# KC-decoder/Multimodal-Brain-Pattern-Identification_XAI

Hardware: AMD Instinct MI355X
Metric: samples/sec train (multimodal SpectrogramCNN+EEGNet fusion, B=64/GPU, 4x128x256 spectro + 10000x19 EEG) (higher is better)
Workload: dtype bf16

## Files before the change

### multimodal-brain-pattern-identification_xai_amd/csrc/conv3x3_mfma.hip

```cpp
#include <stdlib.h>
#include "bx_common.h"
#include <string.h>

typedef __attribute__((ext_vector_type(8))) short bf16x8;
typedef __attribute__((ext_vector_type(4))) float f32x4;
typedef unsigned int u32x4 __attribute__((ext_vector_type(4)));
typedef unsigned int u32x2 __attribute__((ext_vector_type(2)));

static inline int mfma_ck(int Ci) { return Ci < 64 ? Ci : 64; }
static inline int mfma_ks(int ck) { return (9 * ck + 31) / 32; }

int bx_conv3x3_mfma_supported(int Ci, int Co, int dtype) {
  if (dtype != BX_BF16) return 0;
  if (!(Ci == 8 || Ci == 16 || Ci == 32 || (Ci >= 64 && Ci % 64 == 0))) return 0;
  return (Co >= 16 && Co % 16 == 0) || (Co == 8 && (Ci == 16 || Ci == 32));
}
static inline int mfma_ow(int O_p) { return O_p < 16 ? 16 : O_p; }
extern "C" size_t bx_conv3x3_packed_mfma_bytes(int I_p, int O_p) {
  if (!bx_conv3x3_mfma_supported(I_p, O_p, BX_BF16)) return 0;
  const int ck = mfma_ck(I_p);
  return (size_t)(I_p / ck) * mfma_ks(ck) * mfma_ow(O_p) * 32 * sizeof(bf16_t);
}

__global__ void k_pack_mfma(const float* __restrict__ w, bf16_t* __restrict__ wp, int Cout, int Cin, int I_p, int O_p, int tf,
// ... 128 lines not shown
  BX_REQUIRE((src_nchw || src_slot) && dst_nhwc_bf16, "bx_conv3x3_pack_layout_ex: needs a source (pointer or device slot) and a destination");
  BX_REQUIRE(B > 0 && C > 0 && H > 0 && W > 0 && Cp % 8 == 0 && C <= Cp, "bx_conv3x3_pack_layout_ex: Cp must be a multiple of 8 and >= C");
  const long long HW = (long long)H * W;
  const long long nbx = (HW + 255) / 256;
  BX_REQUIRE(HW < (1ll << 31) && nbx * B + total_blocks < (1ll << 31), "bx_conv3x3_pack_layout_ex: input too large");
  hipLaunchKernelGGL(k_pack_mfma_many, dim3((unsigned)(total_blocks + nbx * B)), dim3(256), 0, (hipStream_t)stream, jobs_device, njobs,
                     total_blocks, src_slot ? (const float*)dst_nhwc_bf16  : src_nchw,
                     (bf16_t*)dst_nhwc_bf16, C, Cp, (int)HW, (int)nbx, (uint64_t*)nullptr, (uint64_t*)nullptr, (uint64_t*)nullptr,
                     (uint64_t*)nullptr, src_slot);
  BX_CHECK_LAUNCH("bx_conv3x3_pack_layout_ex");
  return BX_OK;
}
extern "C" int bx_conv3x3_pack_many_step(const bxPackJob* jobs_device, int njobs, int total_blocks, const float* src_nchw, void* dst_nhwc_bf16,
                                         int B, int C, int H, int W, int Cp, uint64_t* state_a, uint64_t* out_a, uint64_t* state_b,
                                         uint64_t* out_b, bxStream stream) {
  BX_REQUIRE(jobs_device && njobs > 0 && total_blocks > 0, "bx_conv3x3_pack_many_step: bad arguments");
  BX_REQUIRE((src_nchw == nullptr) == (dst_nhwc_bf16 == nullptr), "bx_conv3x3_pack_many_step: src and dst go together");
  BX_REQUIRE(state_a && out_a && state_b && out_b && state_a != state_b, "bx_conv3x3_pack_many_step: four seed pointers, two distinct states");
  long long HW = 0, nbx = 1, extra = 0;
  if (src_nchw) {
    BX_REQUIRE(B > 0 && C > 0 && H > 0 && W > 0 && Cp % 8 == 0 && C <= Cp, "bx_conv3x3_pack_many_step: Cp must be a multiple of 8 and >= C");
    HW = (long long)H * W;
    nbx = (HW + 255) / 256;
    extra = nbx * B;
    BX_REQUIRE(HW < (1ll << 31) && extra + total_blocks < (1ll << 31), "bx_conv3x3_pack_many_step: input too large");
  }
  hipLaunchKernelGGL(k_pack_mfma_many, dim3((unsigned)(total_blocks + extra)), dim3(256), 0, (hipStream_t)stream, jobs_device, njobs,
                     total_blocks, src_nchw, (bf16_t*)dst_nhwc_bf16, C, Cp, (int)HW, (int)nbx, state_a, out_a, state_b, out_b);
  BX_CHECK_LAUNCH("bx_conv3x3_pack_many_step");
  return BX_OK;
}

struct WgradRedJob { const float* partial; float* dw; float* db; int nsplit, Cin, Co, S, MA, NB, ztiles, nfrag4, nblocks; };
__device__ __forceinline__ void wgrad_reduce3_body(const WgradRedJob& jb, int bid, float4* sm);
static WgradRedJob wgrad_job_from(const bxWgradPending* pd, bool chained);
#define BX_WGRAD_RED_MAX 3
struct WgradRedList { WgradRedJob job[BX_WGRAD_RED_MAX]; };
__device__ __forceinline__ void wgrad_reduce_list(const WgradRedList& rl, int bid, float4* sm);

template <int CK>
__device__ __forceinline__ int lds_chunk(int c, int p) {
  if (CK == 32) return c ^ ((p >> 1) & 3);
  if (CK == 64) return c ^ (p & 7);
  return c;
}

__device__ __forceinline__ unsigned char relu_bits(u32x2 v) {
  const uint32_t h[4] = {v.x & 0xffffu, v.x >> 16, v.y & 0xffffu, v.y >> 16};
  unsigned b = 0;
#pragma unroll
  for (int r = 0; r < 4; ++r) b |= (h[r] != 0u && h[r] < 0x8000u) ? (1u << r) : 0u;
  return (unsigned char)b;
}
template <int CTRL> __device__ __forceinline__ float dpp16(float v) {
  return __int_as_float(__builtin_amdgcn_update_dpp(0, __float_as_int(v), CTRL, 0xf, 0xf, false));
}
__device__ __forceinline__ float row16_sum(float v) {
  v += dpp16<0xB1>(v); v += dpp16<0x4E>(v); v += dpp16<0x124>(v); v += dpp16<0x128>(v);
  return v;
}
template <int MP, int NC, int TPR, typename PixFn>
__device__ __forceinline__ void conv_pool_tiles(const f32x4 (&q)[MP][NC], const BxConvPoolEpi& pe, const __amdgpu_buffer_rsrc_t& pres, int Co,
                                                int co_base, PixFn pix, float (&st)[2][NC][4]) {
  const int lane = threadIdx.x & 63, g = lane >> 4, li = lane & 15;
  const __amdgpu_buffer_rsrc_t rres = __builtin_amdgcn_make_buffer_rsrc(pe.route, 0, pe.route ? pe.route_bytes : 0u, 0x00020000);
#pragma unroll
// ... 68 lines not shown
  if (bx_stat_tree_arrive<2>(pe.tree, blockIdx.y, co_base, blockIdx.x, val, tot, lds) && (int)threadIdx.x < CW)
    bx_bn_finalize_channel(co_base + threadIdx.x, tot[0], tot[1], pe.fin);
}
__device__ __forceinline__ void conv_pool_transpose_w1x1(const BxConvPoolEpi& pe, int C) {
  const int nw = pe.Cin1_p * C, nwg = (int)(gridDim.x * gridDim.y), wg = (int)(blockIdx.y * gridDim.x + blockIdx.x);
  const int per = (nw + nwg - 1) / nwg, lo = wg * per, hi = lo + per < nw ? lo + per : nw;
  for (int i = lo + (int)threadIdx.x; i < hi; i += 256) {
    const int ci = i / C, c = i - ci * C;
    pe.wT[i] = ci < pe.Cin1 ? pe.w1x1[(size_t)c * pe.Cin1 + ci] : 0.f;
  }
}

#ifdef BX_CONV_STAMPS
__device__ unsigned long long bx_conv_stamps[64 * 8];
extern "C" int bx_debug_conv_stamps(unsigned long long* host_out) {
  return hipMemcpyFromSymbol(host_out, HIP_SYMBOL(bx_conv_stamps), sizeof(unsigned long long) * 64 * 8) == hipSuccess ? 0 : -1;
}
#define BX_CSTAMP(i) do { if (cstamp_wg >= 0 && threadIdx.x == 0) bx_conv_stamps[cstamp_wg * 8 + (i)] = __builtin_amdgcn_s_memtime(); } while (0)
#else
#define BX_CSTAMP(i) do { } while (0)
#endif
template <int CK, int NC, int TW, int IMGS = 1, bool POOL = false, bool C8 = false, bool W22 = false>
__global__ __launch_bounds__(256) void k_conv_mfma(const bf16_t* __restrict__ x, const bf16_t* __restrict__ wp, const float* __restrict__ bias,
    const bf16_t* __restrict__ mask_src, const bf16_t* __restrict__ addend, bf16_t* __restrict__ y,
    int H, int W, int Ci, int Co, int relu, int tiles_x, int tiles_y, uint32_t x_bytes, BxConvPoolEpi pe, WgradRedList red, int nred) {
  constexpr int TH = 8, HWID = TW + 2, HH = TH + 2, CKB = CK * 2, NCH = CK / 8, KS = (9 * CK + 31) / 32;
  constexpr int MP = (W22 ? 2 : 1) * IMGS * TH * TW / 64;
  constexpr int NCW = W22 ? NC / 2 : NC;
  static_assert(!W22 || (NC % 2 == 0 && !POOL && !C8), "2 x 2 wave grid: even NC, plain epilogue");
  constexpr int TPI = TH * TW / 16;
  constexpr int TPR = TW / 16;
  extern __shared__ __attribute__((aligned(16))) char lds[];
  if ((int)blockIdx.x < nred) {
    if (blockIdx.y == 0) wgrad_reduce_list(red, (int)blockIdx.x, reinterpret_cast<float4*>(lds));
    return;
  }
  const int bid = (int)blockIdx.x - nred;
  const int gx = (int)gridDim.x - nred;
#ifdef BX_CONV_STAMPS
  const int cstamp_lin = (int)(blockIdx.y * gridDim.x + blockIdx.x);
  const int cstamp_wg = (cstamp_lin % 4 == 1 && cstamp_lin / 4 < 64) ? cstamp_lin / 4 : -1;
#endif
  BX_CSTAMP(0);
  const int tx = bid % tiles_x, ty = (bid / tiles_x) % tiles_y, b = (bid / (tiles_x * tiles_y)) * IMGS;
  const int wave = threadIdx.x >> 6, lane = threadIdx.x & 63, g = lane >> 4, li = lane & 15;
  const int wpix = W22 ? wave >> 1 : wave;
  const int y0 = ty * TH, x0 = tx * TW, co_base = blockIdx.y * (NC * 16) + (W22 ? (wave & 1) * NCW * 16 : 0);
  if (POOL) conv_pool_transpose_w1x1(pe, Co);

  f32x4 acc[MP][NCW];
#pragma unroll
  for (int i = 0; i < MP; ++i)
#pragma unroll
    for (int n = 0; n < NCW; ++n) acc[i][n] = (f32x4){0.f, 0.f, 0.f, 0.f};

  const int nchunk = Ci / CK;
  const int Cw = C8 ? 16 : Co;
  constexpr int NU = IMGS * HH * HWID * NCH, NR = (NU + 255) / 256;
  const __amdgpu_buffer_rsrc_t xres = __builtin_amdgcn_make_buffer_rsrc((void*)x, 0, x_bytes, 0x00020000);
  uint32_t hoff[NR];
#pragma unroll
  for (int k = 0; k < NR; ++k) {
    const int u = threadIdx.x + k * 256;
    const int p = u / NCH, c = u % NCH;
    const int img = p / (HH * HWID), pl = p - img * (HH * HWID);
    const int iy = y0 + pl / HWID - 1, ix = x0 + pl % HWID - 1;
    const bool ok = u < NU && (unsigned)iy < (unsigned)H && (unsigned)ix < (unsigned)W;
// ... 333 lines not shown
    for (int n = 0; n < NCW; ++n) {
      float v[4] = {acc[i][n][0] + bz[n].x, acc[i][n][1] + bz[n].y, acc[i][n][2] + bz[n].z, acc[i][n][3] + bz[n].w};
      if (relu) {
#pragma unroll
        for (int r = 0; r < 4; ++r) v[r] = fmaxf(v[r], 0.f);
      }
      if (mask_src) {
        const u32x2 m = mk[i][n];
        const uint32_t mm[4] = {m.x & 0xffffu, m.x >> 16, m.y & 0xffffu, m.y >> 16};
#pragma unroll
        for (int r = 0; r < 4; ++r) v[r] = (mm[r] != 0u && mm[r] < 0x8000u) ? v[r] : 0.f;
      }
      if (addend) {
        const u32x2 a2 = ad[i][n];
        v[0] += __uint_as_float(a2.x << 16); v[1] += __uint_as_float(a2.x & 0xffff0000u);
        v[2] += __uint_as_float(a2.y << 16); v[3] += __uint_as_float(a2.y & 0xffff0000u);
      }
      const u32x2 out = {pack2bf(v[0], v[1]), pack2bf(v[2], v[3])};
      __builtin_amdgcn_raw_buffer_store_b64(out, yres, offs[i] + (uint32_t)(n * 32), 0, 0);
    }
  }
  BX_CSTAMP(6);
}

template <int CK, int NC, int TW, bool POOL = false, bool C8 = false>
__global__ __launch_bounds__(256, (CK == 16 && NC == 1 && TW == 32 && !POOL) ? 4 : 1) void k_conv_mfma_p(const bf16_t* __restrict__ x, const bf16_t* __restrict__ wp, const float* __restrict__ bias,
    const bf16_t* __restrict__ mask_src, const bf16_t* __restrict__ addend, bf16_t* __restrict__ y,
    int H, int W, int Co, int relu, int tiles_x, int tiles_y, int ntiles, uint32_t x_bytes, BxConvPoolEpi pe, WgradRedList red, int nred) {
  constexpr int TH = 8, HWID = TW + 2, HH = TH + 2, CKB = CK * 2, NCH = CK / 8, KS = (9 * CK + 31) / 32;
  constexpr int MP = TH * TW / 64, TPR = TW / 16;
  constexpr int NU = HH * HWID * NCH, NR = (NU + 255) / 256;
  extern __shared__ __attribute__((aligned(16))) char lds[];
  if ((int)blockIdx.x < nred) {
    if (blockIdx.y == 0) wgrad_reduce_list(red, (int)blockIdx.x, reinterpret_cast<float4*>(lds));
    return;
  }
  const int first_tile = (int)blockIdx.x - nred, tile_stride = (int)gridDim.x - nred;
  const int co_base = blockIdx.y * (NC * 16);
  const int wave = threadIdx.x >> 6, lane = threadIdx.x & 63, g = lane >> 4, li = lane & 15;
  uint4 rv[NR];
  const __amdgpu_buffer_rsrc_t xres = __builtin_amdgcn_make_buffer_rsrc((void*)x, 0, x_bytes, 0x00020000);
  int hpy[NR], hpx[NR];
  uint32_t hrel[NR];
#pragma unroll
  for (int k = 0; k < NR; ++k) {
    const int u = threadIdx.x + k * 256;
    const int p = u / NCH, c = u % NCH;
    hpy[k] = u < NU ? p / HWID - 1 : -100000;
    hpx[k] = p % HWID - 1;
    hrel[k] = (uint32_t)(((p / HWID - 1) * W + (p % HWID - 1)) * CK + c * 8) * 2u;
  }
  auto fetch = [&](int tile) {
    const int tx = tile % tiles_x, ty = (tile / tiles_x) % tiles_y, b = tile / (tiles_x * tiles_y);
    const int y0 = ty * TH, x0 = tx * TW;
    const uint32_t tbase = (uint32_t)(((b * H + y0) * W + x0) * CK) * 2u;
#pragma unroll
    for (int k = 0; k < NR; ++k) {
      const bool ok = (unsigned)(y0 + hpy[k]) < (unsigned)H && (unsigned)(x0 + hpx[k]) < (unsigned)W;
      const uint32_t off = ok ? tbase + hrel[k] : 0x80000000u;
      const u32x4 v = __builtin_amdgcn_raw_buffer_load_b128(xres, off, 0, 0);
      rv[k] = make_uint4(v.x, v.y, v.z, v.w);
    }
  };
  const uint32_t y_bytes = (uint32_t)((size_t)(ntiles / (tiles_x * tiles_y)) * H * W * Co * 2);
  const __amdgpu_buffer_rsrc_t yres = __builtin_amdgcn_make_buffer_rsrc((void*)y, 0, y_bytes, 0x00020000);
  const bool mbits = (relu & 2) != 0;
  const __amdgpu_buffer_rsrc_t mres = __builtin_amdgcn_make_buffer_rsrc((void*)(mask_src ? mask_src : y), 0, mbits ? y_bytes / 8 : y_bytes, 0x00020000);
// ... 441 lines not shown
  if (y1)
    hipLaunchKernelGGL((k_conv12_mfma<true>), dim3((unsigned)gx), dim3(256), lds, (hipStream_t)stream, (const bf16_t*)x, (const bf16_t*)packed1_mfma, bias1,
                       (const bf16_t*)packed2_mfma, bias2, (bf16_t*)y1, (bf16_t*)y2, mask1, mask2, H, W, tiles_x, tiles_y, (int)ntiles, xb);
  else
    hipLaunchKernelGGL((k_conv12_mfma<false>), dim3((unsigned)gx), dim3(256), lds, (hipStream_t)stream, (const bf16_t*)x, (const bf16_t*)packed1_mfma, bias1,
                       (const bf16_t*)packed2_mfma, bias2, (bf16_t*)nullptr, (bf16_t*)y2, (unsigned char*)nullptr, (unsigned char*)nullptr, H, W, tiles_x, tiles_y, (int)ntiles, xb);
  BX_CHECK_LAUNCH("bx_conv3x3_pair");
  return BX_OK;
}

template <int NC>
static int pool_tree_shape(BxConvPoolEpi* pe, int grid_x, int ygroups, int Co) {
  pe->tree.nrows = grid_x; pe->tree.Cw = NC * 16; pe->tree.ld = Co;
  bx_stat_tree_shape(grid_x, &pe->tree.G, &pe->tree.ngroups);
  if (!pe->want_stats) return BX_OK;
  if (grid_x > pe->tree_max_rows) pe->tree.cnt = nullptr;
  BX_REQUIRE((size_t)grid_x * 2 * Co <= pe->rows_cap_floats, "bx_conv3x3(pooled): %d partial rows exceed the workspace", grid_x);
  BX_REQUIRE(!pe->tree.cnt || ygroups * (pe->tree.ngroups + 1) <= pe->cnt_cap_words, "bx_conv3x3(pooled): %d x %d reduction groups exceed the sync words",
             ygroups, pe->tree.ngroups);
  return BX_OK;
}
static int wgrad_red_total(const WgradRedList& rl) {
  int n = 0;
  for (int i = 0; i < BX_WGRAD_RED_MAX; ++i) n += rl.job[i].nblocks;
  return n;
}
template <int CK, int NC, int TW>
static int launch_conv(const void* x, const void* wp, const float* bias, const void* mask, const void* addend, void* y,
                       int B, int H, int W, int Ci, int Co, int relu, hipStream_t s, BxConvPoolEpi* pe = nullptr, const WgradRedList* red = nullptr) {
  const int tiles_x = (W + TW - 1) / TW, tiles_y = (H + 7) / 8;
  size_t lds = (size_t)10 * (TW + 2) * CK * 2;
  const BxConvPoolEpi none = {};
  const WgradRedList nored = {};
  const int nred = red && !pe ? wgrad_red_total(*red) : 0;
  const WgradRedList& rj = nred ? *red : nored;
  if (nred && lds < 4096) lds = 4096;
  if (pe) {
    const size_t need = BX_STAT_TREE_LDS(2) + (size_t)4 * 2 * NC * 16 * sizeof(float);
    if (lds < need) lds = need;
  }
  if (Co < 16) {
    if constexpr (NC == 1 && (CK == 16 || CK == 32)) {
      BX_REQUIRE(Co == 8 && Ci == CK && !pe && !bias, "bx_conv3x3(mfma): the 8-channel output form is a plain data gradient (Ci=%d Co=%d)", Ci, Co);
      const int ntiles = tiles_x * tiles_y * B;
      const int gx = ntiles < 2048 ? ntiles : 2048;
      if (ntiles >= 4 * gx && (size_t)B * H * W * CK * 2 < ((size_t)1 << 31)) {
        hipLaunchKernelGGL((k_conv_mfma_p<CK, 1, TW, false, true>), dim3((unsigned)(gx + nred), 1u), dim3(256), lds, s, (const bf16_t*)x,
                           (const bf16_t*)wp, bias, (const bf16_t*)mask, (const bf16_t*)addend, (bf16_t*)y, H, W, Co, relu, tiles_x, tiles_y, ntiles,
                           (uint32_t)((size_t)B * H * W * CK * 2), none, rj, nred);
        BX_CHECK_LAUNCH("bx_conv3x3(mfma persistent, 8 output channels)");
        return BX_OK;
      }
      hipLaunchKernelGGL((k_conv_mfma<CK, 1, TW, 1, false, true>), dim3((unsigned)(ntiles + nred), 1u), dim3(256), lds, s, (const bf16_t*)x,
                         (const bf16_t*)wp, bias, (const bf16_t*)mask, (const bf16_t*)addend, (bf16_t*)y, H, W, Ci, Co, relu, tiles_x, tiles_y,
                         (uint32_t)((size_t)B * H * W * Ci * 2), none, rj, nred);
      BX_CHECK_LAUNCH("bx_conv3x3(mfma, 8 output channels)");
      return BX_OK;
    }
    BX_FAIL(BX_EUNSUPPORTED, "bx_conv3x3(mfma): %d output channels with Ci=%d", Co, Ci);
  }
  if constexpr (CK <= 32) if (Ci == CK) {
    const int ntiles = tiles_x * tiles_y * B, ygroups = Co / (16 * NC);
    constexpr int pgx = 2048, pmin = 4;
    int gx = pgx / ygroups;
    if (gx > ntiles) gx = ntiles;
    if (ntiles >= pmin * gx && (size_t)B * H * W * CK * 2 < ((size_t)1 << 31)) {
      if (pe) {
        if constexpr (CK >= 16) {
          const int rc = pool_tree_shape<NC>(pe, gx, ygroups, Co);
          if (rc != BX_OK) return rc;
          hipLaunchKernelGGL((k_conv_mfma_p<CK, NC, TW, true>), dim3((unsigned)gx, (unsigned)ygroups), dim3(256), lds, s, (const bf16_t*)x,
                             (const bf16_t*)wp, bias, (const bf16_t*)nullptr, (const bf16_t*)nullptr, (bf16_t*)y, H, W, Co, 1, tiles_x, tiles_y, ntiles,
                             (uint32_t)((size_t)B * H * W * CK * 2), *pe, nored, 0);
          BX_CHECK_LAUNCH("bx_conv3x3(mfma persistent, pooled)");
          return BX_OK;
        }
      }
      hipLaunchKernelGGL((k_conv_mfma_p<CK, NC, TW>), dim3((unsigned)(gx + nred), (unsigned)ygroups), dim3(256), lds, s, (const bf16_t*)x,
                         (const bf16_t*)wp, bias, (const bf16_t*)mask, (const bf16_t*)addend, (bf16_t*)y, H, W, Co, relu, tiles_x, tiles_y, ntiles,
                         (uint32_t)((size_t)B * H * W * CK * 2), none, rj, nred);
      BX_CHECK_LAUNCH("bx_conv3x3(mfma persistent)");
      return BX_OK;
    }
  }
  if constexpr (CK == 64) {
    if (tiles_x * tiles_y == 1 && Co >= 256 && B % 2 == 0) {
      const size_t lds2 = lds * 2;
      static bool attr_done = false;
      if (lds2 > 64 * 1024 && !attr_done) {
        if (hipFuncSetAttribute((const void*)k_conv_mfma<CK, NC, TW, 2>, hipFuncAttributeMaxDynamicSharedMemorySize, (int)lds2) != hipSuccess)
          BX_FAIL(BX_EHIP, "bx_conv3x3(mfma): cannot reserve %zu bytes of LDS", lds2);
        attr_done = true;
      }
      dim3 grid2((unsigned)(tiles_x * tiles_y * (B / 2) + nred), (unsigned)(Co / (16 * NC)));
      if (pe) {
        const int rc = pool_tree_shape<NC>(pe, (int)grid2.x, (int)grid2.y, Co);
        if (rc != BX_OK) return rc;
        static bool attr_done_p = false;
        if (lds2 > 64 * 1024 && !attr_done_p) {
          if (hipFuncSetAttribute((const void*)k_conv_mfma<CK, NC, TW, 2, true>, hipFuncAttributeMaxDynamicSharedMemorySize, (int)lds2) != hipSuccess)
            BX_FAIL(BX_EHIP, "bx_conv3x3(mfma): cannot reserve %zu bytes of LDS", lds2);
          attr_done_p = true;
        }
        hipLaunchKernelGGL((k_conv_mfma<CK, NC, TW, 2, true>), grid2, dim3(256), lds2, s, (const bf16_t*)x, (const bf16_t*)wp, bias, (const bf16_t*)nullptr,
                           (const bf16_t*)nullptr, (bf16_t*)y, H, W, Ci, Co, 1, tiles_x, tiles_y, (uint32_t)((size_t)B * H * W * Ci * 2), *pe, nored, 0);
        BX_CHECK_LAUNCH("bx_conv3x3(mfma, two-image tiles, pooled)");
        return BX_OK;
      }
      hipLaunchKernelGGL((k_conv_mfma<CK, NC, TW, 2>), grid2, dim3(256), lds2, s, (const bf16_t*)x, (const bf16_t*)wp, bias, (const bf16_t*)mask,
                         (const bf16_t*)addend, (bf16_t*)y, H, W, Ci, Co, relu, tiles_x, tiles_y, (uint32_t)((size_t)B * H * W * Ci * 2), none, rj, nred);
      BX_CHECK_LAUNCH("bx_conv3x3(mfma, two-image tiles)");
      return BX_OK;
    }
  }
  dim3 grid((unsigned)(tiles_x * tiles_y * B + nred), (unsigned)(Co / (16 * NC)));
  if (pe) {
    if constexpr (CK >= 16) {
      const int rc = pool_tree_shape<NC>(pe, (int)grid.x, (int)grid.y, Co);
      if (rc != BX_OK) return rc;
      hipLaunchKernelGGL((k_conv_mfma<CK, NC, TW, 1, true>), grid, dim3(256), lds, s, (const bf16_t*)x, (const bf16_t*)wp, bias, (const bf16_t*)nullptr,
                         (const bf16_t*)nullptr, (bf16_t*)y, H, W, Ci, Co, 1, tiles_x, tiles_y, (uint32_t)((size_t)B * H * W * Ci * 2), *pe, nored, 0);
      BX_CHECK_LAUNCH("bx_conv3x3(mfma, pooled)");
      return BX_OK;
    }
    BX_FAIL(BX_EUNSUPPORTED, "bx_conv3x3(pooled): needs at least 16 input channels");
  }
  if constexpr (CK == 64 && NC % 2 == 0) {
    hipLaunchKernelGGL((k_conv_mfma<CK, NC, TW, 1, false, false, true>), grid, dim3(256), lds, s, (const bf16_t*)x, (const bf16_t*)wp, bias,
                       (const bf16_t*)mask, (const bf16_t*)addend, (bf16_t*)y, H, W, Ci, Co, relu, tiles_x, tiles_y, (uint32_t)((size_t)B * H * W * Ci * 2), none, rj, nred);
    BX_CHECK_LAUNCH("bx_conv3x3(mfma, 2 x 2 waves)");
  } else {
    hipLaunchKernelGGL((k_conv_mfma<CK, NC, TW>), grid, dim3(256), lds, s, (const bf16_t*)x, (const bf16_t*)wp, bias,
                       (const bf16_t*)mask, (const bf16_t*)addend, (bf16_t*)y, H, W, Ci, Co, relu, tiles_x, tiles_y, (uint32_t)((size_t)B * H * W * Ci * 2), none, rj, nred);
    BX_CHECK_LAUNCH("bx_conv3x3(mfma)");
  }
  return BX_OK;
}
template <int NCW, int TW, int IMGS>
static int launch_conv_c(const void* x, const void* wp, const float* bias, const void* mask, const void* addend, void* y,
                         int B, int H, int W, int Ci, int Co, int relu, hipStream_t s, BxConvPoolEpi* pe) {
  const int tiles_x = (W + TW - 1) / TW, tiles_y = (H + 7) / 8;
  const size_t lds = (size_t)2 * IMGS * 10 * ((TW + 2 + 7) / 8 * 8) * 128;
  dim3 grid((unsigned)(tiles_x * tiles_y * (B / IMGS)), (unsigned)(Co / (64 * NCW)));
  const BxConvPoolEpi none = {};
  auto attr = [&](const void* fn, bool& done) -> int {
    if (lds > 64 * 1024 && !done) {
      if (hipFuncSetAttribute(fn, hipFuncAttributeMaxDynamicSharedMemorySize, (int)lds) != hipSuccess)
// ... 61 lines not shown
  for (int i = 0, k = 0; carry && i < ncarry; ++i)
    if (carry[i].valid) { jobs.job[k++] = wgrad_job_from(&carry[i], true); red = &jobs; }
  BX_REQUIRE((size_t)B * H * W * (Ci > Co ? Ci : Co) * 2 < ((size_t)1 << 31), "bx_conv3x3(mfma): an activation tensor of 2 GiB or more is not supported (B=%d H=%d W=%d)", B, H, W);
  if (!red) {
    const int rc = try_conv_c(x, packed_mfma, bias, relu_mask_src, addend, y, B, H, W, Ci, Co, relu, s, nullptr);
    if (rc >= 0) return rc;
  }
  int rc;
  switch (mfma_ck(Ci)) {
    case 8:  rc = launch_conv_nc<8>(x, packed_mfma, bias, relu_mask_src, addend, y, B, H, W, Ci, Co, relu, s, nullptr, red); break;
    case 16: rc = launch_conv_nc<16>(x, packed_mfma, bias, relu_mask_src, addend, y, B, H, W, Ci, Co, relu, s, nullptr, red); break;
    case 32: rc = launch_conv_nc<32>(x, packed_mfma, bias, relu_mask_src, addend, y, B, H, W, Ci, Co, relu, s, nullptr, red); break;
    default: rc = launch_conv_nc<64>(x, packed_mfma, bias, relu_mask_src, addend, y, B, H, W, Ci, Co, relu, s, nullptr, red); break;
  }
  for (int i = 0; rc == BX_OK && carry && i < ncarry; ++i) carry[i].valid = 0;
  return rc;
}

int bx_conv3x3_mfma_pool_launch(const void* x, const void* packed_mfma, const float* bias, void* y, int B, int H, int W, int Ci, int Co,
                                BxConvPoolEpi* pe, hipStream_t s) {
  BX_REQUIRE((size_t)B * H * W * (Ci > Co ? Ci : Co) * 2 < ((size_t)1 << 31), "bx_conv3x3(pooled): an activation tensor of 2 GiB or more is not supported");
  BX_REQUIRE(Ci >= 16 && pe && pe->pooled, "bx_conv3x3(pooled): needs at least 16 input channels and a pooled output");
  {
    const int rc = try_conv_c(x, packed_mfma, bias, nullptr, nullptr, y, B, H, W, Ci, Co, 1, s, pe);
    if (rc >= 0) return rc;
  }
  switch (mfma_ck(Ci)) {
    case 16: return launch_conv_nc<16>(x, packed_mfma, bias, nullptr, nullptr, y, B, H, W, Ci, Co, 1, s, pe);
    case 32: return launch_conv_nc<32>(x, packed_mfma, bias, nullptr, nullptr, y, B, H, W, Ci, Co, 1, s, pe);
    default: return launch_conv_nc<64>(x, packed_mfma, bias, nullptr, nullptr, y, B, H, W, Ci, Co, 1, s, pe);
  }
}

__device__ __forceinline__ void wgrad_reduce3_body(const WgradRedJob& jb, int bid, float4* sm) {
  const float* __restrict__ partial = jb.partial;
  float* __restrict__ dw = jb.dw;
  float* __restrict__ db = jb.db;
  const int nsplit = jb.nsplit, Cin = jb.Cin, Co = jb.Co, S = jb.S, MA = jb.MA, NB = jb.NB, ztiles = jb.ztiles, nfrag4 = jb.nfrag4;
  const size_t per_split = (size_t)nfrag4 * 4 + Co;
  const int NO = 256 / S;
  const int o = threadIdx.x % NO, part = threadIdx.x / NO;
  const size_t e4 = (size_t)bid * NO + o;
  const bool live = e4 * 4 < per_split;
  float4 s = make_float4(0.f, 0.f, 0.f, 0.f);
  if (live) {
    const float* src = partial + e4 * 4;
    int c = part;
    for (; c + 3 * S < nsplit; c += 4 * S) {
      const float4 v0 = *reinterpret_cast<const float4*>(src + (size_t)c * per_split);
      const float4 v1 = *reinterpret_cast<const float4*>(src + (size_t)(c + S) * per_split);
      const float4 v2 = *reinterpret_cast<const float4*>(src + (size_t)(c + 2 * S) * per_split);
      const float4 v3 = *reinterpret_cast<const float4*>(src + (size_t)(c + 3 * S) * per_split);
      s.x += v0.x; s.y += v0.y; s.z += v0.z; s.w += v0.w;
      s.x += v1.x; s.y += v1.y; s.z += v1.z; s.w += v1.w;
      s.x += v2.x; s.y += v2.y; s.z += v2.z; s.w += v2.w;
      s.x += v3.x; s.y += v3.y; s.z += v3.z; s.w += v3.w;
    }
    for (; c < nsplit; c += S) {
      const float4 v = *reinterpret_cast<const float4*>(src + (size_t)c * per_split);
      s.x += v.x; s.y += v.y; s.z += v.z; s.w += v.w;
    }
  }
  sm[threadIdx.x] = s;
  __syncthreads();
  if (part == 0 && live) {
    float4 r = sm[o];
    for (int k = 1; k < S; ++k) { const float4 v = sm[k * NO + o]; r.x += v.x; r.y += v.y; r.z += v.z; r.w += v.w; }
    const float rr[4] = {r.x, r.y, r.z, r.w};
    if (e4 < (size_t)nfrag4) {
      const int NT = 9 * MA * NB;
      const int lane = (int)(e4 & 63), tl = (int)(e4 >> 6);
      const int i = tl % NT, yz = tl / NT, z = yz % ztiles, y = yz / ztiles;
      const int n = i % NB, m = (i / NB) % MA, t = i / (NB * MA);
      const int cout = (z * NB + n) * 16 + (lane & 15), cin0 = (y * MA + m) * 16 + 4 * (lane >> 4);
#pragma unroll
      for (int j = 0; j < 4; ++j)
        if (cin0 + j < Cin) dw[((size_t)cout * Cin + cin0 + j) * 9 + t] = rr[j];
    } else if (db) {
      const size_t b0 = (e4 - nfrag4) * 4;
#pragma unroll
      for (int j = 0; j < 4; ++j) db[b0 + j] = rr[j];
    }
  }
}
__device__ __forceinline__ void wgrad_reduce_list(const WgradRedList& rl, int bid, float4* sm) {
  if (bid < rl.job[0].nblocks) { wgrad_reduce3_body(rl.job[0], bid, sm); return; }
  bid -= rl.job[0].nblocks;
  if (bid < rl.job[1].nblocks) { wgrad_reduce3_body(rl.job[1], bid, sm); return; }
  bid -= rl.job[1].nblocks;
  if (bid < rl.job[2].nblocks) wgrad_reduce3_body(rl.job[2], bid, sm);
}
__global__ __launch_bounds__(256) void k_wgrad_reduce3(WgradRedJob jb, WgradRedJob jb2) {
  __shared__ float4 sm[256];
  if ((int)blockIdx.x < jb.nblocks) wgrad_reduce3_body(jb, blockIdx.x, sm);
  else wgrad_reduce3_body(jb2, (int)blockIdx.x - jb.nblocks, sm);
}

typedef __attribute__((ext_vector_type(4))) short s16x4;
typedef __attribute__((address_space(3))) s16x4 lds_s16x4;

__device__ __forceinline__ bf16x8 tr_read8(const char* lds, int off0, int off1) {
  const s16x4 lo = __builtin_amdgcn_ds_read_tr16_b64_v4i16((lds_s16x4*)(lds + off0));
  const s16x4 hi = __builtin_amdgcn_ds_read_tr16_b64_v4i16((lds_s16x4*)(lds + off1));
  return (bf16x8){lo[0], lo[1], lo[2], lo[3], hi[0], hi[1], hi[2], hi[3]};
}

template <int MA, int NB, int TW>
__global__ __launch_bounds__(256, 2) void k_wgrad_mfma(const bf16_t* __restrict__ x, const bf16_t* __restrict__ dz, float* __restrict__ partial,
    int H, int W, int Ci_p, int Co, int tiles_x, int tiles_y, int ntiles, int tiles_per_split, WgradRedJob prev, int zextra) {
  constexpr int TH = 8, HWID = TW + 2, HH = TH + 2, CIT = 16 * MA, COT = 16 * NB, XB = CIT * 2, ZB = COT * 2;
  constexpr int KPW = TH * TW / 32 / 4;
  constexpr int XS_BYTES = HH * HWID * XB;
  extern __shared__ __attribute__((aligned(16))) char lds[];
  if ((int)blockIdx.z < zextra) {
    const int rid = ((int)blockIdx.z * (int)gridDim.y + (int)blockIdx.y) * (int)gridDim.x + (int)blockIdx.x;
    if (rid < prev.nblocks) wgrad_reduce3_body(prev, rid, reinterpret_cast<float4*>(lds));
    return;
  }
  const int bz = (int)blockIdx.z - zextra, gz = (int)gridDim.z - zextra;
  char* xs = lds;
  char* zs = lds + XS_BYTES;
  const int wave = threadIdx.x >> 6, lane = threadIdx.x & 63, g = lane >> 4, li = lane & 15;
  const int q = li >> 2, pc = li & 3;
  const int ci0 = blockIdx.y * CIT, co0 = bz * COT;
  const bool want_bias = blockIdx.y == 0;

// ... 348 lines not shown
  wgrad_own_body<TW>(*pj, id - pj->first, lds);
}

struct WgradPlan { int ma, nb, tw, tiles_x, tiles_y, ntiles, ytiles, ztiles, nsplit, tps; size_t lds; };
static WgradPlan wgrad_plan(int B, int H, int W, int Ci_p, int Co) {
  WgradPlan p;
  p.ma = Ci_p >= 32 ? 2 : 1;
  p.nb = Co >= 32 ? 2 : 1;
  p.tw = W <= 16 ? 16 : 32;
  p.tiles_x = (W + p.tw - 1) / p.tw; p.tiles_y = (H + 7) / 8; p.ntiles = p.tiles_x * p.tiles_y * B;
  p.ytiles = (Ci_p + 16 * p.ma - 1) / (16 * p.ma); p.ztiles = Co / (16 * p.nb);
  constexpr int want_wgs = 512;
  int want = want_wgs / (p.ytiles * p.ztiles);
  if (want < 1) want = 1;
  if (want > p.ntiles) want = p.ntiles;
  p.tps = (p.ntiles + want - 1) / want;
  p.nsplit = (p.ntiles + p.tps - 1) / p.tps;
  const size_t stage = (size_t)10 * (p.tw + 2) * 32 * p.ma + (size_t)8 * p.tw * 32 * p.nb;
  const size_t red = (size_t)((9 * p.ma * p.nb + 3) / 4) * 4 * 64 * sizeof(float4);
  p.lds = stage > red ? stage : red;
  return p;
}
int bx_wgrad_mfma_supported(int Ci_p, int Co, int dtype) {
  return dtype == BX_BF16 && Ci_p % 8 == 0 && Co % 16 == 0 && (Co < 32 || Co % 32 == 0) && (Ci_p < 32 || Ci_p % 32 == 0);
}
size_t bx_wgrad_mfma_workspace(int B, int H, int W, int Ci_p, int Co) {
  const WgradPlan p = wgrad_plan(B, H, W, Ci_p, Co);
  return (size_t)p.nsplit * ((size_t)p.ytiles * p.ztiles * 9 * p.ma * p.nb * 256 + Co) * sizeof(float);
}
template <int MA, int NB, int TW>
static void launch_wgrad(const WgradPlan& p, const void* x, const void* dz, float* ws, int H, int W, int Ci_p, int Co, const WgradRedJob& prev,
                         int zextra, hipStream_t s) {
  dim3 grid(p.nsplit, p.ytiles, p.ztiles + zextra);
  hipLaunchKernelGGL((k_wgrad_mfma<MA, NB, TW>), grid, dim3(256), p.lds, s, (const bf16_t*)x, (const bf16_t*)dz, ws, H, W, Ci_p, Co,
                     p.tiles_x, p.tiles_y, p.ntiles, p.tps, prev, zextra);
}
static int wgrad_reduce_slices(size_t per_split, int nsplit, bool chained) {
  if (!chained) return per_split >= 65536 ? 4 : per_split >= 8192 ? 16 : 64;
  int S = 1;
  while (S < 64 && nsplit > 8 * S) S *= 2;
  return S;
}
static WgradRedJob wgrad_job_from(const bxWgradPending* pd, bool chained) {
  WgradRedJob jb;
  jb.partial = (const float*)pd->partial; jb.dw = pd->dw; jb.db = pd->db; jb.nsplit = pd->nsplit; jb.Cin = pd->Cin; jb.Co = pd->Co;
  jb.MA = pd->ma; jb.NB = pd->nb; jb.ztiles = pd->ztiles; jb.nfrag4 = pd->nfrag4;
  const size_t per_split = (size_t)pd->nfrag4 * 4 + pd->Co;
  jb.S = wgrad_reduce_slices(per_split, pd->nsplit, chained);
  const int per_wg = 256 / jb.S;
  jb.nblocks = (int)((per_split / 4 + per_wg - 1) / per_wg);
  return jb;
}
int bx_wgrad_mfma_finish(bxWgradPending* pd, hipStream_t s) {
  if (!pd || !pd->valid) return BX_OK;
  const WgradRedJob jb = wgrad_job_from(pd, false), none = {};
  hipLaunchKernelGGL(k_wgrad_reduce3, dim3(jb.nblocks), dim3(256), 0, s, jb, none);
  pd->valid = 0;
  BX_CHECK_LAUNCH("bx_conv3x3_wgrad(mfma reduce)");
  return BX_OK;
}
int bx_wgrad_mfma_launch(const void* x, const void* dz, float* dw, float* db, int B, int H, int W, int Cin, int Ci_p,
                         int Co, void* ws, size_t ws_bytes, bxWgradPending* pending, hipStream_t s) {
  const WgradPlan p = wgrad_plan(B, H, W, Ci_p, Co);
  (void)ws_bytes;
  BX_REQUIRE((size_t)B * H * W * (Ci_p > Co ? Ci_p : Co) * 2 < ((size_t)1 << 31), "bx_conv3x3_wgrad(mfma): an activation tensor of 2 GiB or more is not supported");
  BX_REQUIRE(!pending || !pending->valid || pending->partial != ws, "bx_conv3x3_wgrad(chained): the pending partials live in this call's workspace");
  float* part = (float*)ws;
  WgradRedJob prev;
  memset(&prev, 0, sizeof(prev));
  int zextra = 0;
  if (pending && pending->valid) {
    prev = wgrad_job_from(pending, true);
    zextra = (prev.nblocks + p.nsplit * p.ytiles - 1) / (p.nsplit * p.ytiles);
  }
  if (p.ma == 2 && p.nb == 2) {
    const int nred = pending && pending->valid ? (prev.nblocks + 7) / 8 * 8 : 0;
    const int ranges8 = (p.nsplit + 7) / 8;
    const int nwg = nred + ranges8 * 8 * p.ytiles * p.ztiles;
    const size_t lds = (size_t)10 * (p.tw + 2) * 64 + (size_t)8 * p.tw * 64 + 256;
    if (p.tw == 16)
      hipLaunchKernelGGL((k_wgrad_own<16, 2>), dim3(nwg), dim3(256), lds, s, (const bf16_t*)x, (const bf16_t*)dz, part, H, W, Ci_p, Co,
                         p.tiles_x, p.tiles_y, p.ntiles, p.tps, p.nsplit, p.ytiles, p.ztiles, prev, nred);
    else
      hipLaunchKernelGGL((k_wgrad_own<32, 2>), dim3(nwg), dim3(256), lds, s, (const bf16_t*)x, (const bf16_t*)dz, part, H, W, Ci_p, Co,
                         p.tiles_x, p.tiles_y, p.ntiles, p.tps, p.nsplit, p.ytiles, p.ztiles, prev, nred);
  } else {
#define BX_WG(MA_, NB_) do { if (p.tw == 16) launch_wgrad<MA_, NB_, 16>(p, x, dz, part, H, W, Ci_p, Co, prev, zextra, s); \
                             else launch_wgrad<MA_, NB_, 32>(p, x, dz, part, H, W, Ci_p, Co, prev, zextra, s); } while (0)
    if (p.ma == 1 && p.nb == 1) BX_WG(1, 1);
    else if (p.ma == 1) BX_WG(1, 2);
    else BX_WG(2, 1);
#undef BX_WG
  }
  BX_CHECK_LAUNCH("bx_conv3x3_wgrad(mfma)");
  bxWgradPending cur;
  cur.partial = part; cur.dw = dw; cur.db = db; cur.nsplit = p.nsplit; cur.Cin = Cin; cur.Co = Co; cur.ma = p.ma; cur.nb = p.nb;
  cur.ztiles = p.ztiles; cur.nfrag4 = p.ytiles * p.ztiles * 9 * p.ma * p.nb * 64; cur.valid = 1;
  if (pending) { *pending = cur; return BX_OK; }
  return bx_wgrad_mfma_finish(&cur, s);
}

static size_t wgrad_group_region(size_t bytes) { return (bytes + 255) / 256 * 256; }
int bx_wgrad_group_supported(int n, const int* Ci_p, const int* Co, int W, int dtype) {
  if (n < 1 || n > BX_WGRAD_GROUP_MAX || !Ci_p || !Co || W <= 0 || dtype != BX_BF16) return 0;
  for (int i = 0; i < n; ++i)
    if (Ci_p[i] < 32 || Co[i] < 32 || !bx_wgrad_mfma_supported(Ci_p[i], Co[i], dtype)) return 0;
  return 1;
}
size_t bx_wgrad_group_workspace(const bxWgradGroupLayer* layers, int n, int B, int H, int W) {
  size_t total = 0;
  for (int i = 0; i < n; ++i) total += wgrad_group_region(bx_wgrad_mfma_workspace(B, H, W, layers[i].Ci_p, layers[i].Co));
  return total;
// ... 246 lines not shown
}

struct FusedBwdPlan { int tiles_x, tiles_y, ntiles, tps, nsplit; };
static FusedBwdPlan fused_bwd_plan(int B, int H, int W) {
  FusedBwdPlan p;
  p.tiles_x = (W + 31) / 32; p.tiles_y = (H + 7) / 8; p.ntiles = p.tiles_x * p.tiles_y * B;
  constexpr int want_wgs = 512;
  const int want = want_wgs < p.ntiles ? want_wgs : p.ntiles;
  p.tps = (p.ntiles + want - 1) / want;
  p.nsplit = (p.ntiles + p.tps - 1) / p.tps;
  return p;
}
extern "C" size_t bx_conv3x3_bwd_fused_workspace(int B, int H, int W, int with_w1) {
  const FusedBwdPlan p = fused_bwd_plan(B, H, W);
  return (size_t)p.nsplit * (9 * 256 + 16) * sizeof(float) * (with_w1 ? 2 : 1);
}
extern "C" int bx_conv3x3_bwd_fused(const void* dz, const void* xl, const void* packed_flip, void* dzo, const void* x0, float* dw, float* db,
                                    float* dw0, float* db0, int B, int H, int W, int Cin0, void* ws, size_t ws_bytes, bxWgradPending* pending,
                                    bxStream stream) {
  hipStream_t s = (hipStream_t)stream;
  const bool w1 = x0 != nullptr;
  BX_REQUIRE(dz && xl && packed_flip && dw && db && ws && B > 0 && H > 0 && W > 0, "bx_conv3x3_bwd_fused: bad arguments");
  BX_REQUIRE(w1 ? (!dzo && dw0 && db0 && Cin0 > 0 && Cin0 <= 8) : (dzo && !dw0 && !db0),
             "bx_conv3x3_bwd_fused: either dzo (data gradient stored) or x0 with dw0 / db0 (conv1's weight gradient, 1..8 input channels)");
  BX_REQUIRE((size_t)B * H * W * 16 * 2 < ((size_t)1 << 31), "bx_conv3x3_bwd_fused: an activation tensor of 2 GiB or more is not supported");
  const FusedBwdPlan p = fused_bwd_plan(B, H, W);
  const size_t need = bx_conv3x3_bwd_fused_workspace(B, H, W, w1);
  BX_REQUIRE(ws_bytes >= need, "bx_conv3x3_bwd_fused: workspace %zu < %zu", ws_bytes, need);
  BX_REQUIRE(!pending || !pending->valid || pending->partial != ws, "bx_conv3x3_bwd_fused: the pending partials live in this call's workspace");
  WgradRedJob prev = {};
  int nred = 0;
  if (pending && pending->valid) { prev = wgrad_job_from(pending, true); nred = prev.nblocks; pending->valid = 0; }
  constexpr int IMG = 10 * 34 * 32;
  const size_t lds = w1 ? (size_t)3 * IMG + 8 * 32 * 32 : (size_t)2 * IMG;
  const uint32_t act_bytes = (uint32_t)((size_t)B * H * W * 16 * 2);
  float* part = (float*)ws;
  if (w1)
    hipLaunchKernelGGL((k_conv_mfma_bwd<true>), dim3((unsigned)(p.nsplit + nred)), dim3(256), lds, s, (const bf16_t*)dz, (const bf16_t*)xl,
                       (const bf16_t*)packed_flip, (const bf16_t*)x0, (bf16_t*)nullptr, part, H, W, p.tiles_x, p.tiles_y, p.ntiles, p.tps, p.nsplit,
                       act_bytes, prev, nred);
  else
    hipLaunchKernelGGL((k_conv_mfma_bwd<false>), dim3((unsigned)(p.nsplit + nred)), dim3(256), lds, s, (const bf16_t*)dz, (const bf16_t*)xl,
                       (const bf16_t*)packed_flip, (const bf16_t*)nullptr, (bf16_t*)dzo, part, H, W, p.tiles_x, p.tiles_y, p.ntiles, p.tps, p.nsplit,
                       act_bytes, prev, nred);
  BX_CHECK_LAUNCH("bx_conv3x3_bwd_fused");
  bxWgradPending cur = {};
  cur.partial = part; cur.dw = dw; cur.db = db; cur.nsplit = p.nsplit; cur.Cin = 16; cur.Co = 16; cur.ma = 1; cur.nb = 1;
  cur.ztiles = 1; cur.nfrag4 = 9 * 64; cur.valid = 1;
  if (!w1) {
    if (pending) { *pending = cur; return BX_OK; }
    return bx_wgrad_mfma_finish(&cur, s);
  }
  bxWgradPending cur0 = cur;
  cur0.partial = part + (size_t)p.nsplit * (9 * 256 + 16); cur0.dw = dw0; cur0.db = db0; cur0.Cin = Cin0;
  const WgradRedJob j1 = wgrad_job_from(&cur, false), j0 = wgrad_job_from(&cur0, false);
  hipLaunchKernelGGL(k_wgrad_reduce3, dim3((unsigned)(j1.nblocks + j0.nblocks)), dim3(256), 0, s, j1, j0);
  BX_CHECK_LAUNCH("bx_conv3x3_bwd_fused(reduce)");
  return BX_OK;
}
```

Before: 48990.

## Reduce wgrad partials per tap triplet and spread reduction blocks across grid y

Adds a new reduction path for small split counts: each thread sums three taps of a fragment position across splits, stages the results in LDS, and then writes dw in the final Co×Ci×3×3 layout with coalesced float4 stores, replacing the old scattered per-element writes. Fused conv launches now spread the chained reduction blocks over every grid-y row instead of only row 0, which shortens the idle x-prefix of the grid. LDS reservations are raised wherever a chained reduction runs. The cost is more LDS per block, which can lower occupancy for small conv kernels, plus extra synchronization inside the reduction.

```diff
diff --git a/multimodal-brain-pattern-identification_xai_amd/csrc/conv3x3_mfma.hip b/multimodal-brain-pattern-identification_xai_amd/csrc/conv3x3_mfma.hip
--- a/multimodal-brain-pattern-identification_xai_amd/csrc/conv3x3_mfma.hip
+++ b/multimodal-brain-pattern-identification_xai_amd/csrc/conv3x3_mfma.hip
@@ -184,6 +184,7 @@
 }
 
 struct WgradRedJob { const float* partial; float* dw; float* db; int nsplit, Cin, Co, S, MA, NB, ztiles, nfrag4, nblocks; };
+#define BX_WGRAD_RED_LDS ((size_t)3 * 256 * sizeof(float4) + (size_t)85 * 36 * sizeof(float))
 __device__ __forceinline__ void wgrad_reduce3_body(const WgradRedJob& jb, int bid, float4* sm);
 static WgradRedJob wgrad_job_from(const bxWgradPending* pd, bool chained);
 #define BX_WGRAD_RED_MAX 3
@@ -318,7 +319,7 @@
   constexpr int TPR = TW / 16;
   extern __shared__ __attribute__((aligned(16))) char lds[];
   if ((int)blockIdx.x < nred) {
-    if (blockIdx.y == 0) wgrad_reduce_list(red, (int)blockIdx.x, reinterpret_cast<float4*>(lds));
+    if constexpr (!POOL) wgrad_reduce_list(red, (int)(blockIdx.y * nred + blockIdx.x), reinterpret_cast<float4*>(lds));
     return;
   }
   const int bid = (int)blockIdx.x - nred;
@@ -718,7 +719,7 @@
   constexpr int NU = HH * HWID * NCH, NR = (NU + 255) / 256;
   extern __shared__ __attribute__((aligned(16))) char lds[];
   if ((int)blockIdx.x < nred) {
-    if (blockIdx.y == 0) wgrad_reduce_list(red, (int)blockIdx.x, reinterpret_cast<float4*>(lds));
+    wgrad_reduce_list(red, (int)(blockIdx.y * nred + blockIdx.x), reinterpret_cast<float4*>(lds));
     return;
   }
   const int first_tile = (int)blockIdx.x - nred, tile_stride = (int)gridDim.x - nred;
@@ -1226,9 +1227,10 @@
   size_t lds = (size_t)10 * (TW + 2) * CK * 2;
   const BxConvPoolEpi none = {};
   const WgradRedList nored = {};
-  const int nred = red && !pe ? wgrad_red_total(*red) : 0;
-  const WgradRedList& rj = nred ? *red : nored;
-  if (nred && lds < 4096) lds = 4096;
+  const int nblk = red && !pe ? wgrad_red_total(*red) : 0;
+  const auto nredx = [nblk](int ny) { return (nblk + ny - 1) / ny; };
+  const WgradRedList& rj = nblk ? *red : nored;
+  if (nblk && lds < BX_WGRAD_RED_LDS) lds = BX_WGRAD_RED_LDS;
   if (pe) {
     const size_t need = BX_STAT_TREE_LDS(2) + (size_t)4 * 2 * NC * 16 * sizeof(float);
     if (lds < need) lds = need;
@@ -1236,7 +1238,7 @@
   if (Co < 16) {
     if constexpr (NC == 1 && (CK == 16 || CK == 32)) {
       BX_REQUIRE(Co == 8 && Ci == CK && !pe && !bias, "bx_conv3x3(mfma): the 8-channel output form is a plain data gradient (Ci=%d Co=%d)", Ci, Co);
-      const int ntiles = tiles_x * tiles_y * B;
+      const int ntiles = tiles_x * tiles_y * B, nred = nredx(1);
       const int gx = ntiles < 2048 ? ntiles : 2048;
       if (ntiles >= 4 * gx && (size_t)B * H * W * CK * 2 < ((size_t)1 << 31)) {
         hipLaunchKernelGGL((k_conv_mfma_p<CK, 1, TW, false, true>), dim3((unsigned)(gx + nred), 1u), dim3(256), lds, s, (const bf16_t*)x,
@@ -1254,7 +1256,7 @@
     BX_FAIL(BX_EUNSUPPORTED, "bx_conv3x3(mfma): %d output channels with Ci=%d", Co, Ci);
   }
   if constexpr (CK <= 32) if (Ci == CK) {
-    const int ntiles = tiles_x * tiles_y * B, ygroups = Co / (16 * NC);
+    const int ntiles = tiles_x * tiles_y * B, ygroups = Co / (16 * NC), nred = nredx(ygroups);
     constexpr int pgx = 2048, pmin = 4;
     int gx = pgx / ygroups;
     if (gx > ntiles) gx = ntiles;
@@ -1286,6 +1288,7 @@
           BX_FAIL(BX_EHIP, "bx_conv3x3(mfma): cannot reserve %zu bytes of LDS", lds2);
         attr_done = true;
       }
+      const int nred = nredx(Co / (16 * NC));
       dim3 grid2((unsigned)(tiles_x * tiles_y * (B / 2) + nred), (unsigned)(Co / (16 * NC)));
       if (pe) {
         const int rc = pool_tree_shape<NC>(pe, (int)grid2.x, (int)grid2.y, Co);
@@ -1307,6 +1310,7 @@
       return BX_OK;
     }
   }
+  const int nred = nredx(Co / (16 * NC));
   dim3 grid((unsigned)(tiles_x * tiles_y * B + nred), (unsigned)(Co / (16 * NC)));
   if (pe) {
     if constexpr (CK >= 16) {
@@ -1434,7 +1438,8 @@
   }
 }
 
-__device__ __forceinline__ void wgrad_reduce3_body(const WgradRedJob& jb, int bid, float4* sm) {
+#define BX_WGRAD_POS_MAX_S 4
+__device__ __forceinline__ void wgrad_reduce3_runs(const WgradRedJob& jb, int bid, float4* sm) {
   const float* __restrict__ partial = jb.partial;
   float* __restrict__ dw = jb.dw;
   float* __restrict__ db = jb.db;
@@ -1485,6 +1490,88 @@
     }
   }
 }
+__device__ __forceinline__ void wgrad_reduce3_body(const WgradRedJob& jb, int bid, float4* sm) {
+  if (jb.S > BX_WGRAD_POS_MAX_S) { wgrad_reduce3_runs(jb, bid, sm); return; }
+  const float* __restrict__ partial = jb.partial;
+  float* __restrict__ dw = jb.dw;
+  float* __restrict__ db = jb.db;
+  const int nsplit = jb.nsplit, Cin = jb.Cin, Co = jb.Co, S = jb.S, MA = jb.MA, NB = jb.NB, ztiles = jb.ztiles, nfrag4 = jb.nfrag4;
+  const size_t per_split = (size_t)nfrag4 * 4 + Co;
+  const int NO = 256 / S, NP = NO / 3, MN = MA * NB, P = nfrag4 / 9;
+  const int idx = threadIdx.x % NO, part = threadIdx.x / NO;
+  const int tg = idx / NP, pl = idx % NP;
+  const int q = bid * NP + pl;
+  const bool frag = tg < 3 && q < P, bias = tg == 0 && q >= P && (q - P) * 4 < Co;
+  float* stage = reinterpret_cast<float*>(sm + 3 * 256);
+  float acc[3][4];
+#pragma unroll
+  for (int t = 0; t < 3; ++t)
+#pragma unroll
+    for (int j = 0; j < 4; ++j) acc[t][j] = 0.f;
+  if (frag) {
+    const int lane = q & 63, mn = (q >> 6) % MN, yz = (q >> 6) / MN;
+    const size_t tap_stride = (size_t)MN * 256;
+    const float* src = partial + (((size_t)yz * 9 * MN + mn) * 64 + lane) * 4 + 3 * tg * tap_stride;
+#pragma unroll 1
+    for (int c = part; c < nsplit; c += S) {
+      const float* p0 = src + (size_t)c * per_split;
+      float4 v[3];
+#pragma unroll
+      for (int t = 0; t < 3; ++t) v[t] = *reinterpret_cast<const float4*>(p0 + t * tap_stride);
+#pragma unroll
+      for (int t = 0; t < 3; ++t) { acc[t][0] += v[t].x; acc[t][1] += v[t].y; acc[t][2] += v[t].z; acc[t][3] += v[t].w; }
+    }
+  } else if (bias) {
+    const float* src = partial + ((size_t)nfrag4 + (q - P)) * 4;
+    for (int c = part; c < nsplit; c += S) {
+      const float4 v = *reinterpret_cast<const float4*>(src + (size_t)c * per_split);
+      acc[0][0] += v.x; acc[0][1] += v.y; acc[0][2] += v.z; acc[0][3] += v.w;
+    }
+  }
+  if (S > 1) {
+#pragma unroll
+    for (int t = 0; t < 3; ++t) sm[t * 256 + threadIdx.x] = make_float4(acc[t][0], acc[t][1], acc[t][2], acc[t][3]);
+    __syncthreads();
+    if (part == 0 && (frag || bias))
+#pragma unroll 2
+      for (int k = 1; k < S; ++k) {
+#pragma unroll
+        for (int t = 0; t < 3; ++t) {
+          const float4 v = sm[t * 256 + k * NO + idx];
+          acc[t][0] += v.x; acc[t][1] += v.y; acc[t][2] += v.z; acc[t][3] += v.w;
+        }
+      }
+  }
+  if (part == 0 && frag) {
+#pragma unroll
+    for (int t = 0; t < 3; ++t)
+#pragma unroll
+      for (int j = 0; j < 4; ++j) stage[pl * 36 + j * 9 + 3 * tg + t] = acc[t][j];
+  } else if (part == 0 && bias && db) {
+    const int b0 = (q - P) * 4;
+#pragma unroll
+    for (int j = 0; j < 4; ++j) db[b0 + j] = acc[0][j];
+  }
+  __syncthreads();
+  const int q0 = bid * NP, npos = P - q0 < NP ? P - q0 : NP;
+#pragma unroll 1
+  for (int u = threadIdx.x; u < npos * 9; u += 256) {
+    const int up = u / 9, k = u % 9, qq = q0 + up;
+    const int lane = qq & 63, mn = (qq >> 6) % MN, yz = (qq >> 6) / MN;
+    const int z = yz % ztiles, y = yz / ztiles, n = mn % NB, m = mn / NB;
+    const int cout = (z * NB + n) * 16 + (lane & 15), cin0 = (y * MA + m) * 16 + 4 * (lane >> 4);
+    float* dst = dw + ((size_t)cout * Cin + cin0) * 9 + 4 * k;
+    const float4 v = *reinterpret_cast<const float4*>(stage + up * 36 + 4 * k);
+    if (cin0 + 4 <= Cin && ((size_t)dst & 15) == 0) {
+      *reinterpret_cast<float4*>(dst) = v;
+    } else {
+      const float vv[4] = {v.x, v.y, v.z, v.w};
+#pragma unroll
+      for (int i = 0; i < 4; ++i)
+        if (cin0 + (4 * k + i) / 9 < Cin) dst[i] = vv[i];
+    }
+  }
+}
 __device__ __forceinline__ void wgrad_reduce_list(const WgradRedList& rl, int bid, float4* sm) {
   if (bid < rl.job[0].nblocks) { wgrad_reduce3_body(rl.job[0], bid, sm); return; }
   bid -= rl.job[0].nblocks;
@@ -1493,7 +1580,7 @@
   if (bid < rl.job[2].nblocks) wgrad_reduce3_body(rl.job[2], bid, sm);
 }
 __global__ __launch_bounds__(256) void k_wgrad_reduce3(WgradRedJob jb, WgradRedJob jb2) {
-  __shared__ float4 sm[256];
+  __shared__ float4 sm[BX_WGRAD_RED_LDS / sizeof(float4)];
   if ((int)blockIdx.x < jb.nblocks) wgrad_reduce3_body(jb, blockIdx.x, sm);
   else wgrad_reduce3_body(jb2, (int)blockIdx.x - jb.nblocks, sm);
 }
@@ -1908,7 +1995,8 @@
 static void launch_wgrad(const WgradPlan& p, const void* x, const void* dz, float* ws, int H, int W, int Ci_p, int Co, const WgradRedJob& prev,
                          int zextra, hipStream_t s) {
   dim3 grid(p.nsplit, p.ytiles, p.ztiles + zextra);
-  hipLaunchKernelGGL((k_wgrad_mfma<MA, NB, TW>), grid, dim3(256), p.lds, s, (const bf16_t*)x, (const bf16_t*)dz, ws, H, W, Ci_p, Co,
+  const size_t lds = zextra && p.lds < BX_WGRAD_RED_LDS ? BX_WGRAD_RED_LDS : p.lds;
+  hipLaunchKernelGGL((k_wgrad_mfma<MA, NB, TW>), grid, dim3(256), lds, s, (const bf16_t*)x, (const bf16_t*)dz, ws, H, W, Ci_p, Co,
                      p.tiles_x, p.tiles_y, p.ntiles, p.tps, prev, zextra);
 }
 static int wgrad_reduce_slices(size_t per_split, int nsplit, bool chained) {
@@ -1923,8 +2011,13 @@
   jb.MA = pd->ma; jb.NB = pd->nb; jb.ztiles = pd->ztiles; jb.nfrag4 = pd->nfrag4;
   const size_t per_split = (size_t)pd->nfrag4 * 4 + pd->Co;
   jb.S = wgrad_reduce_slices(per_split, pd->nsplit, chained);
-  const int per_wg = 256 / jb.S;
-  jb.nblocks = (int)((per_split / 4 + per_wg - 1) / per_wg);
+  if (jb.S > BX_WGRAD_POS_MAX_S) {
+    const int per_wg = 256 / jb.S;
+    jb.nblocks = (int)((per_split / 4 + per_wg - 1) / per_wg);
+  } else {
+    const int per_wg = 256 / jb.S / 3;
+    jb.nblocks = (pd->nfrag4 / 9 + pd->Co / 4 + per_wg - 1) / per_wg;
+  }
   return jb;
 }
 int bx_wgrad_mfma_finish(bxWgradPending* pd, hipStream_t s) {
@@ -1953,7 +2046,8 @@
     const int nred = pending && pending->valid ? (prev.nblocks + 7) / 8 * 8 : 0;
     const int ranges8 = (p.nsplit + 7) / 8;
     const int nwg = nred + ranges8 * 8 * p.ytiles * p.ztiles;
-    const size_t lds = (size_t)10 * (p.tw + 2) * 64 + (size_t)8 * p.tw * 64 + 256;
+    size_t lds = (size_t)10 * (p.tw + 2) * 64 + (size_t)8 * p.tw * 64 + 256;
+    if (nred && lds < BX_WGRAD_RED_LDS) lds = BX_WGRAD_RED_LDS;
     if (p.tw == 16)
       hipLaunchKernelGGL((k_wgrad_own<16, 2>), dim3(nwg), dim3(256), lds, s, (const bf16_t*)x, (const bf16_t*)dz, part, H, W, Ci_p, Co,
                          p.tiles_x, p.tiles_y, p.ntiles, p.tps, p.nsplit, p.ytiles, p.ztiles, prev, nred);
@@ -2266,7 +2360,8 @@
   int nred = 0;
   if (pending && pending->valid) { prev = wgrad_job_from(pending, true); nred = prev.nblocks; pending->valid = 0; }
   constexpr int IMG = 10 * 34 * 32;
-  const size_t lds = w1 ? (size_t)3 * IMG + 8 * 32 * 32 : (size_t)2 * IMG;
+  size_t lds = w1 ? (size_t)3 * IMG + 8 * 32 * 32 : (size_t)2 * IMG;
+  if (nred && lds < BX_WGRAD_RED_LDS) lds = BX_WGRAD_RED_LDS;
   const uint32_t act_bytes = (uint32_t)((size_t)B * H * W * 16 * 2);
   float* part = (float*)ws;
   if (w1)
```

Result: no change. 49190 (median of 2 runs) (+0.4%).
